# flanglet/kanzi

Hardware: AMD Instinct MI355X
Metric: encode+decode MB/s, 4 MiB-block synthetic stream, BWT+RANK+ZRLT & ANS0 (level-5 core chain), bit-exact .knz (higher is better)
Workload: dtype u8; 1 GPU; configs[2]: BWT+RANK+ZRLT & ANS0, 2048 x 4194304 B blocks per GPU per step (64 distinct synthetic blocks per GPU, SURVEY 8d generator standing in for silesia.tar, tiled), blocks round-robin over ranks; block_size=4194304, parallelism=blocks%1, round_trip_ok=True

## Files before the change

kanzi_amd/csrc/kz_ans.hip:

```cpp
#include "kz_device.h"
#include "kz_internal.h"
#include "kz_chunk.h"

typedef uint16_t u16;

#define ANS_TOP (1u << 15)
#define ANS_LR 12


struct BitW { u8* p; u32 pos; };
__device__ __forceinline__ void bw_put(BitW& w, u32 v, int count) {
  while (count > 0) {
    const int bitoff = w.pos & 7, room = 8 - bitoff;
    const int take = count < room ? count : room;
    const u32 bits = (v >> (count - take)) & ((1u << take) - 1u);
    w.p[w.pos >> 3] |= (u8)(bits << (room - take));
    w.pos += take; count -= take;
  }
}

typedef u16 __attribute__((aligned(1))) ans_u16_unaligned;
typedef u64 __attribute__((aligned(1))) ans_u64_unaligned;

__global__ __launch_bounds__(64) void k_ans_enc_chunk(const u8* __restrict__ src, int64_t stride,
                                                       const int32_t* __restrict__ d_len, AnsEnc E) {
  const int b = blockIdx.y, ck = blockIdx.x;
  const int count = d_len[b];
  const int lane = kz_lane();
  const int64_t ci = (int64_t)b * E.C + ck;
  const u8* blk = src + (int64_t)b * stride;
  u8* hdr = E.hdr + ci * ANS_HDR_BYTES;
  u8* scr = E.scr + ci * ANS_SCRATCH;
  if (count <= 32) {
    if (ck != 0) return;
    if (lane < count) scr[lane] = blk[lane];
    if (lane == 0) { E.hdrBits[ci] = 0; E.tailOff[ci] = 0; E.tailBits[ci] = 8u * (u32)count; }
    return;
  }
  const int start = ck * ANS_CHUNK;
  if (start >= count) return;
  const int end = min(count, start + ANS_CHUNK);
  const int len = end - start;

  __shared__ u32 hist[256];
  __shared__ u16 nfreq[256];
  __shared__ u8 alpha[256];
  __shared__ uint4 symTab[256];
  const u8* data = blk + start;
  __shared__ u32 hbuf[ANS_HDR_BYTES / 4];

  for (int i = lane; i < 256; i += 64) hist[i] = 0;
  for (int i = lane; i < ANS_HDR_BYTES / 4; i += 64) hbuf[i] = 0;
  __syncthreads();
  for (int i = lane * 4; i < len; i += 256) {
    u32 w = 0; int nb = min(4, len - i);
    if (nb == 4 && ((start + i) & 3) == 0) w = *(const u32*)(blk + start + i);
    else for (int k = 0; k < nb; k++) w |= (u32)blk[start + i + k] << (8 * k);
    for (int k = 0; k < 4; k++) {
      const bool valid = k < nb;
      const u32 c = (w >> (8 * k)) & 0xFF;
      const uint64_t peers = kz_match8(c, valid);
      if (valid && (peers & kz_lanemask_lt()) == 0) atomicAdd(&hist[c], (u32)__popcll(peers));
    }
  }
  __syncthreads();

  const u32 total = (u32)len, scale = 1u << ANS_LR;
  u32 f[4]; bool present[4];
  u32 alphabetSize = 0;
  u32 apos[4];
#pragma unroll
  for (int q = 0; q < 4; q++) {
    f[q] = hist[q * 64 + lane];
    present[q] = f[q] != 0;
    const uint64_t bal = kz_ballot(present[q]);
    apos[q] = alphabetSize + (u32)__popcll(bal & kz_lanemask_lt());
    alphabetSize += (u32)__popcll(bal);
    if (present[q]) alpha[apos[q]] = (u8)(q * 64 + lane);
  }
  if (total != scale) {
    u32 sumScaled = 0;
#pragma unroll
    for (int q = 0; q < 4; q++) {
      if (present[q]) {
        const u32 sf = f[q] * scale;
        f[q] = (sf <= total) ? 1u : (sf + (total >> 1)) / total;
      }
      sumScaled += kz_wave_sum(present[q] ? f[q] : 0);
    }
    if (alphabetSize == 1) {
#pragma unroll
      for (int q = 0; q < 4; q++) if (present[q]) f[q] = scale;
    } else if (sumScaled != scale) {
      u32 best = 0;
#pragma unroll
      for (int q = 0; q < 4; q++) { u32 v = present[q] ? f[q] : 0; best = max(best, v); }
#pragma unroll
      for (int d = 32; d > 0; d >>= 1) best = max(best, (u32)__shfl_xor(best, d, 64));
      int idxMax = 256;
#pragma unroll
      for (int q = 3; q >= 0; q--) {
        const uint64_t bal = kz_ballot(present[q] && f[q] == best);
        if (bal) idxMax = q * 64 + (int)__builtin_ctzll(bal);
      }
      int delta = (int)sumScaled - (int)scale;
      const int errThr = (int)(best >> 4);
      const int mq = idxMax >> 6, ml = idxMax & 63;
      int adjMax = 0;
      const int ad = delta < 0 ? -delta : delta;
      if (ad <= errThr) {
        adjMax = -delta;
      } else {
        if (delta < 0) { delta += errThr; adjMax = errThr; } else { delta -= errThr; adjMax = -errThr; }
#pragma unroll
        for (int q = 0; q < 4; q++) if (q == mq && lane == ml) f[q] = (u32)((int)f[q] + adjMax);
        adjMax = 0;
        const int inc = (delta > 0) ? -1 : 1;
        delta = delta < 0 ? -delta : delta;
        int round = 0;
        while ((++round < 6) && (delta > 0)) {
          int adjustments = 0;
#pragma unroll
          for (int q = 0; q < 4; q++) {
            const bool elig = present[q] && f[q] > 2;
            const uint64_t bal = kz_ballot(elig);
            const int pre = (int)__popcll(bal & kz_lanemask_lt());
            const int tot = (int)__popcll(bal);
            if (elig && pre < delta) f[q] = (u32)((int)f[q] + inc);
            const int used = tot < delta ? tot : delta;
            adjustments += used; delta -= used;
          }
          if (adjustments == 0) break;
        }
#pragma unroll
        for (int q = 0; q < 4; q++) if (q == mq && lane == ml) { int v = (int)f[q] - delta; f[q] = (u32)(v > 1 ? v : 1); }
      }
      if (adjMax != 0) {
#pragma unroll
        for (int q = 0; q < 4; q++) if (q == mq && lane == ml) f[q] = (u32)((int)f[q] + adjMax);
      }
    }
  }
  u32 cum = 0;
#pragma unroll
  for (int q = 0; q < 4; q++) {
    const u32 fv = present[q] ? f[q] : 0;
    const u32 inc = kz_wave_incl_sum(fv);
    const u32 cumFreq = cum + inc - fv;
    cum += __shfl(inc, 63, 64);
    const int s = q * 64 + lane;
    nfreq[s] = (u16)fv;
    if (present[q]) {
      u32 freq = fv;
      if (freq >= scale) freq = scale - 1;
      const u32 xmaxv = ((ANS_TOP >> ANS_LR) << 16) * freq;
      const u32 cmplv = scale - freq;
      if (freq < 2) symTab[s] = make_uint4(xmaxv, 0xFFFFFFFFu, cumFreq + scale - 1, cmplv | (32u << 16));
      else {
        int shift = 0;
        while (freq > (1u << shift)) shift++;
        symTab[s] = make_uint4(xmaxv, (u32)((((1ULL << (shift + 31)) + freq - 1) / freq) & 0xFFFFFFFFULL), cumFreq, cmplv | ((u32)(32 + shift - 1) << 16));
      }
    }
  }
  __syncthreads();
  u32 hb = 0;
  if (lane == 0) {
    BitW w{(u8*)hbuf, 0};
    bw_put(w, ANS_LR - 8, 3);
    if (alphabetSize == 256) { bw_put(w, 0, 1); bw_put(w, 0, 1); }
    else if (alphabetSize == 0) { bw_put(w, 0, 1); bw_put(w, 1, 1); }
    else {
      bw_put(w, 1, 1);
      const int lastMask = alpha[alphabetSize - 1] >> 3;
      bw_put(w, (u32)lastMask, 5);
      for (int i = 0; i <= lastMask; i++) {
        u32 m = 0;
        for (int j = 0; j < 8; j++) if (nfreq[i * 8 + j] != 0) m |= 1u << j;
        bw_put(w, m, 8);
      }
    }
    if (alphabetSize > 1) {
      const int chkSize = (alphabetSize >= 64) ? 8 : 6;
      int llr = 3;
      while ((1 << llr) <= ANS_LR) llr++;
      for (int i = 1; i < (int)alphabetSize; i += chkSize) {
        const int endj = (i + chkSize < (int)alphabetSize) ? i + chkSize : (int)alphabetSize;
        int mx = (int)nfreq[alpha[i]] - 1;
        for (int j = i + 1; j < endj; j++) { int v = (int)nfreq[alpha[j]] - 1; if (v > mx) mx = v; }
        int logMax = 0;
        while ((1 << logMax) <= mx) logMax++;
        bw_put(w, (u32)logMax, llr);
        if (logMax == 0) continue;
        for (int j = i; j < endj; j++) bw_put(w, (u32)nfreq[alpha[j]] - 1u, logMax);
      }
    }
    hb = w.pos;
    E.hdrBits[ci] = hb;
  }
  __syncthreads();
  for (int i = lane; i < ANS_HDR_BYTES / 4; i += 64) ((u32*)hdr)[i] = hbuf[i];
  if (alphabetSize <= 1) {
    if (lane == 0) { E.tailOff[ci] = 0; E.tailBits[ci] = 0; }
    return;
  }
  const int bufLen = ANS_SCRATCH;
  const int end4 = len & -4;
  int n = bufLen - 1;
  if (lane == 0) for (int i = len - 1; i >= end4; i--) scr[n - (len - 1 - i)] = data[i];
  n -= (len - end4);
  u32 st = ANS_TOP;
  int idx = n;
  if (lane < 4) {
#define ANS_ENC_STEP(WD)                                                                                      \
    { const u32 c = ((WD) >> (8 * (3 - lane))) & 0xFFu;                                                       \
      const uint4 sy = symTab[c];                                                                             \
      const bool x = st >= sy.x;                                               \
      const uint64_t bal = kz_ballot(x) & 0xFULL;                                                             \
      const int pre = (int)__popcll(bal & kz_lanemask_lt());                                                  \
      if (x) {                                                       \
        const int e = idx - 2 * pre;                                                                          \
        *(ans_u16_unaligned*)(scr + e - 1) = (u16)(((st & 0xFFu) << 8) | ((st >> 8) & 0xFFu));                \
        st >>= 16;                                                                                            \
      }                                                                                                       \
      idx -= 2 * (int)__popcll(bal);                                                                          \
      const u32 q = (u32)(((u64)st * (u64)sy.y) >> (sy.w >> 16));                                             \
      st = st + sy.z + q * (sy.w & 0xFFFFu); }
    const int T = end4 >> 2;
    const uint4* d16 = (const uint4*)data;
    int g = (T - 1) >> 2;
    uint4 cur = (T > 0) ? d16[g] : make_uint4(0, 0, 0, 0);
    for (; g >= 0; g--) {
      const uint4 nxt = (g > 0) ? d16[g - 1] : make_uint4(0, 0, 0, 0);
      const int top = min(3, T - 1 - 4 * g);
      if (top >= 3) ANS_ENC_STEP(cur.w)
      if (top >= 2) ANS_ENC_STEP(cur.z)
      if (top >= 1) ANS_ENC_STEP(cur.y)
      ANS_ENC_STEP(cur.x)
      cur = nxt;
    }
#undef ANS_ENC_STEP
  }
  idx = __shfl(idx, 0, 64);
  n = idx + 1;
  const u32 payload = (u32)(bufLen - n);
  u32 vlen = 1; { u32 v = payload; while (v >= 128) { v >>= 7; vlen++; } }
  const int tail = n - 16 - (int)vlen;
  if (lane == 0) {
    u32 v = payload; int p = tail;
    while (v >= 128) { scr[p++] = (u8)(0x80 | (v & 0x7F)); v >>= 7; }
    scr[p++] = (u8)v;
    E.tailOff[ci] = (u32)tail; E.tailBits[ci] = 8u * (payload + 16 + vlen);
  }
  if (lane < 4) {
    u8* p = scr + tail + vlen + 4 * lane;
    p[0] = (u8)(st >> 24); p[1] = (u8)(st >> 16); p[2] = (u8)(st >> 8); p[3] = (u8)st;
  }
}

__global__ __launch_bounds__(64) void k_ans_enc_scan(const int32_t* __restrict__ d_len, AnsEnc E, int64_t* __restrict__ d_bits, int rawLimit) {
  const int b = blockIdx.x;
  const int count = d_len[b];
  const int chunks = (count <= rawLimit) ? (count > 0 ? 1 : 0) : (count + E.chunk - 1) / E.chunk;
  const int lane = kz_lane();
  u64 carry = 0;
  for (int base = 0; base < chunks; base += 64) {
    const int c = base + lane;
    const int64_t ci = (int64_t)b * E.C + c;
    const u32 v = (c < chunks) ? E.hdrBits[ci] + E.tailBits[ci] : 0;
    const u32 inc = kz_wave_incl_sum(v);
    if (c < chunks) E.bitOff[ci] = carry + inc - v;
    carry += __shfl(inc, 63, 64);
  }
  if (lane == 0) d_bits[b] = (int64_t)carry;
}

__device__ __forceinline__ u32 kz_fetch32(const u8* __restrict__ p, int64_t nbits, int64_t r) {
  if (r >= nbits || r + 32 <= 0) return 0;
  u64 acc = 0;
  const int64_t byte0 = (r >= 0) ? (r >> 3) : -((-r + 7) >> 3);
  const int64_t nbytes = (nbits + 7) >> 3;
#pragma unroll
  for (int k = 0; k < 5; k++) {
    const int64_t bi = byte0 + k;
    const u64 v = (bi >= 0 && bi < nbytes) ? p[bi] : 0;
    acc = (acc << 8) | v;
  }
  const int sh = (int)(r - byte0 * 8);
  u32 w = (u32)((acc << sh) >> 8);
  const int64_t over = r + 32 - nbits;
  if (over > 0) w &= (over >= 32) ? 0u : (0xFFFFFFFFu << over);
  if (r < 0) { const int64_t under = -r; w &= (under >= 32) ? 0u : (0xFFFFFFFFu >> under); }
  return w;
}

__global__ __launch_bounds__(KZ_WG) void k_ans_enc_concat(const int32_t* __restrict__ d_len, AnsEnc E, u8* __restrict__ out,
                                                           int64_t outStride, const int32_t* __restrict__ d_hdrBytes, int rawLimit) {
  const int b = blockIdx.y, ck = blockIdx.x;
  const int count = d_len[b];
  const int chunks = (count <= rawLimit) ? (count > 0 ? 1 : 0) : (count + E.chunk - 1) / E.chunk;
  if (ck >= chunks) return;
  const int64_t ci = (int64_t)b * E.C + ck;
  const u8* hdr = E.hdr + ci * E.hdrStride;
  const int64_t hb = E.hdrBits[ci];
  const int64_t tb = (int64_t)E.tailBits[ci];
  const u8* tail = E.scr + ci * E.scrStride + E.tailOff[ci];
  const int64_t len = hb + tb;
  if (len == 0) return;
  const int64_t base = 8LL * d_hdrBytes[b] + (int64_t)E.bitOff[ci];
  u32* o = (u32*)(out + (int64_t)b * outStride);
  const int64_t wEnd = (base + len - 1) >> 5, wCap = (E.outCap >> 2) - 1;
  const int64_t w0 = base >> 5, w1 = wEnd < wCap ? wEnd : wCap;
  for (int64_t w = w0 + threadIdx.x; w <= w1; w += KZ_WG) {
    const int64_t r = w * 32 - base;
    u32 v = kz_fetch32(hdr, hb, r) | kz_fetch32(tail, tb, r - hb);
    v = __builtin_bswap32(v);
    if (r >= 0 && r + 32 <= len) o[w] = v; else atomicOr(&o[w], v);
  }
}

size_t kz_ans_scratch(int B, int maxN) {
  const int C = (maxN + 64) / ANS_CHUNK + 2;
  return (size_t)B * C * (ANS_HDR_BYTES + ANS_SCRATCH + 32) + (size_t)B * 64 + 8192;
}

int kz_chunk_enc_alloc(kz_ctx* ctx, kz_batch& bt, AnsEnc& E, int* chunksOut) {
  const int B = bt.B;
  int maxN = 0;
  for (int b = 0; b < B; b++) if (bt.h_len[b] > maxN) maxN = bt.h_len[b];
  E.C = (maxN + ANS_CHUNK - 1) / ANS_CHUNK + 1;
  E.hdr = (u8*)kz_arena_alloc(ctx, (size_t)B * E.C * ANS_HDR_BYTES);
  E.scr = (u8*)kz_arena_alloc(ctx, (size_t)B * E.C * ANS_SCRATCH);
  E.hdrBits = (u32*)kz_arena_alloc(ctx, (size_t)B * E.C * 4);
  E.tailOff = (u32*)kz_arena_alloc(ctx, (size_t)B * E.C * 4);
  E.tailBits = (u32*)kz_arena_alloc(ctx, (size_t)B * E.C * 4);
  E.bitOff = (u64*)kz_arena_alloc(ctx, (size_t)B * E.C * 8);
  if (!E.bitOff || !E.scr) { snprintf(ctx->err, sizeof(ctx->err), "entropy encode: arena overflow"); return -KZ_ERR_DEVICE; }
  KZ_HIP(hipMemsetAsync(E.hdrBits, 0, (size_t)B * E.C * 4, ctx->stream));
  KZ_HIP(hipMemsetAsync(E.tailBits, 0, (size_t)B * E.C * 4, ctx->stream));
  *chunksOut = (maxN + ANS_CHUNK - 1) / ANS_CHUNK;
  return 0;
}
int kz_chunk_enc_finish(kz_ctx* ctx, kz_batch& bt, AnsEnc& E, int chunks, uint8_t* out, int64_t outStride,
                        const int32_t* d_hdrBytes, int64_t* d_bits, int rawLimit) {
  const int B = bt.B;
  KZ_LAUNCH(ctx, KID_ANS_ENC_SCAN, k_ans_enc_scan, dim3(B), dim3(64), bt.d_len, E, d_bits, rawLimit);
  if (chunks > 0) KZ_LAUNCH(ctx, KID_ANS_ENC_CONCAT, k_ans_enc_concat, dim3(chunks, B), dim3(KZ_WG), bt.d_len, E, out, outStride, d_hdrBytes, rawLimit);
  KZ_HIP(hipGetLastError());
  return 0;
}

int kz_stage_ans0_encode(kz_ctx* ctx, kz_batch& bt, uint8_t* out, int64_t outStride, const int32_t* d_hdrBytes, int64_t* d_bits) {
  AnsEnc E; int chunks = 0;
  int rc = kz_chunk_enc_alloc(ctx, bt, E, &chunks);
  if (rc) return rc;
  if (chunks > 0) KZ_LAUNCH(ctx, KID_ANS_ENC_CHUNK, k_ans_enc_chunk, dim3(chunks, bt.B), dim3(64), bt.buf[bt.cur], bt.stride, bt.d_len, E);
  return kz_chunk_enc_finish(ctx, bt, E, chunks, out, outStride, d_hdrBytes, d_bits, 32);
}

#define ANS_EV_NONE 0x7FFFFFFF
#define ANS_EV_FAIL 0
#define ANS_EV_SKIP 1
#define ANS_EV_STOP 2
#define ANS_MAX_CHUNK_SIZE (1u << 27)
struct AnsDec {
  u64* chunkBit;
  int32_t* event;
  int32_t* nIdx;
  int32_t* hdrOnly;
  int C;
};

__device__ __forceinline__ u32 kz_peek(const u8* __restrict__ p, u64 pos, int count) {
  const u64 by = pos >> 3;
  u32 acc = ((u32)p[by] << 24) | ((u32)p[by + 1] << 16) | ((u32)p[by + 2] << 8) | (u32)p[by + 3];
  acc <<= (pos & 7);
  return count ? (acc >> (32 - count)) : 0;
}

__global__ void k_ans_dec_index(const u8* __restrict__ in, int64_t inStride, const int64_t* __restrict__ d_bitOff,
                                const int64_t* __restrict__ d_bitEnd, const int32_t* __restrict__ d_len, AnsDec D, int B, long long* __restrict__ endOut) {
  const int b = blockIdx.x * blockDim.x + threadIdx.x;
  if (b >= B) return;
  const int count = d_len[b];
  const u8* p = in + (int64_t)b * inStride;
  u64 pos = (u64)d_bitOff[b];
  const u64 endBits = (u64)d_bitEnd[b];
  int event = ANS_EV_NONE, nIdx = 0, bufLen = 0, hdrOnly = -1;
  if (count > 32) {
    const int chunks = (count + ANS_CHUNK - 1) / ANS_CHUNK;
    for (int c = 0; c < chunks; c++) {
      D.chunkBit[(int64_t)b * D.C + c] = pos;
      if (pos + 5 > endBits) { event = c * 4 + ANS_EV_FAIL; break; }
      const int lr = 8 + (int)kz_peek(p, pos, 3); pos += 3;
      int asz;
      if (kz_peek(p, pos, 1) == 0) { asz = (kz_peek(p, pos + 1, 1) == 1) ? 0 : 256; pos += 2; }
      else {
        const int lastMask = (int)kz_peek(p, pos + 1, 5); pos += 6;
        asz = 0;
        if (pos + 8ULL * (u64)(lastMask + 1) > endBits) { event = c * 4 + ANS_EV_FAIL; break; }
        for (int i = 0; i <= lastMask; i++) { asz += __popc(kz_peek(p, pos, 8)); pos += 8; }
      }
      if (asz == 0) { event = c * 4 + ANS_EV_FAIL; break; }
      {
        const int chkSize = (asz >= 64) ? 8 : 6;
        int llr = 3;
        while ((1 << llr) <= lr) llr++;
        for (int i = 1; i < asz && pos <= endBits; i += chkSize) {
          const int logMax = (int)kz_peek(p, pos, llr); pos += llr;
          const int endj = (i + chkSize < asz) ? i + chkSize : asz;
          pos += (u64)logMax * (u64)(endj - i);
        }
      }
      if (pos > endBits) { event = c * 4 + ANS_EV_FAIL; break; }
      nIdx = c + 1;
      if (asz == 1) continue;
      u32 v = kz_peek(p, pos, 8); pos += 8;
      u32 sz = v & 0x7F; int shift = 7;
      while (v >= 128) { v = kz_peek(p, pos, 8); pos += 8; sz |= (v & 0x7F) << shift; if (shift == 28) break; shift += 7; }
      if (sz >= ANS_MAX_CHUNK_SIZE) { hdrOnly = c; event = c * 4 + ANS_EV_SKIP; break; }
      const int clen = min(count - c * ANS_CHUNK, ANS_CHUNK);
      bufLen = max(bufLen, max(2 * clen, 256));
      if (sz > (u32)bufLen) { nIdx = c; event = c * 4 + ANS_EV_FAIL; break; }
      pos += 128 + 8ULL * sz;
      if (pos > endBits) { nIdx = c; event = c * 4 + ANS_EV_FAIL; break; }
    }
    if (event == ANS_EV_NONE) D.chunkBit[(int64_t)b * D.C + chunks] = pos;
  } else {
    pos += 8ULL * (u64)(count > 0 ? count : 0);
    if (pos > endBits) event = ANS_EV_FAIL;
  }
  if (endOut) endOut[b] = (long long)pos;
  D.event[b] = event;
  D.nIdx[b] = nIdx;
  D.hdrOnly[b] = hdrOnly;
}

__device__ __forceinline__ void ans_fill_f2s(const u16* __restrict__ cumf, u8* __restrict__ f2s, int scale, int lane) {
  const int x0 = lane * 64;
// ... 197 lines not shown
```

kanzi_amd/csrc/kz_api.hip:

```cpp
#include <dirent.h>
#include "kz_device.h"
#include "kz_internal.h"
#include <stdlib.h>
#include <algorithm>
#include <atomic>
#include <memory>
#include <thread>
#include <chrono>
#include <sched.h>

typedef uint32_t u32;
typedef uint8_t u8;
typedef unsigned long long u64;

extern "C" int32_t kz_abi_version(void) { return KZ_ABI_VERSION; }

extern "C" kz_ctx* kz_ctx_create(int32_t deviceId) {
  int ndev = 0;
  if (hipGetDeviceCount(&ndev) != hipSuccess || ndev <= 0) return nullptr;
  if (deviceId < 0 || deviceId >= ndev) return nullptr;
  if (hipSetDevice(deviceId) != hipSuccess) return nullptr;
  kz_ctx* ctx = new kz_ctx();
  ctx->device = deviceId;
  { int cus = 0; if (hipDeviceGetAttribute(&cus, hipDeviceAttributeMultiprocessorCount, deviceId) == hipSuccess && cus > 0) ctx->numCUs = cus; }
  if (hipStreamCreateWithFlags(&ctx->stream, hipStreamNonBlocking) != hipSuccess) { delete ctx; return nullptr; }
  if (hipHostMalloc((void**)&ctx->hpin, 1 << 20, hipHostMallocDefault) != hipSuccess) { hipStreamDestroy(ctx->stream); delete ctx; return nullptr; }
  ctx->hpinInts = (1 << 20) / 4;
  kz_switches_read(ctx->sw);
  {
    const int hw = (int)std::thread::hardware_concurrency();
    ctx->blockingWaits = ctx->sw.blockingWaits >= 0 ? ctx->sw.blockingWaits : ((hw > 0 && kz_usable_cpus() < hw) ? 1 : 0);
  }
  return ctx;
}
void kz_switches_read(kz_switches& s) {
  s = kz_switches();
  auto num = [](const char* name, int unset) { const char* e = getenv(name); return e ? atoi(e) : unset; };
  auto flag = [](const char* name) { return getenv(name) != nullptr ? 1 : 0; };
  auto digit = [](const char* name, int lo, int hi, int unset) { const char* e = getenv(name); return (e && e[0] >= '0' + lo && e[0] <= '0' + hi) ? e[0] - '0' : unset; };
  { const char* e = getenv("KZ_BLOCKING_WAITS"); s.blockingWaits = e ? (atoi(e) ? 1 : 0) : -1; }
  s.textGpu = digit("KZ_TEXT_GPU", 0, 3, -1);
  s.textGpuMin = num("KZ_TEXT_GPU_MIN", 512);
  s.textFwdGpu = digit("KZ_TEXT_FWD_GPU", 0, 1, -1);
  s.textFwdGpuMin = num("KZ_TEXT_FWD_GPU_MIN", 256);
  s.utfGpu = digit("KZ_UTF_GPU", 0, 0, 1);
  s.utfFwdGpu = digit("KZ_UTF_FWD_GPU", 0, 1, -1);
  s.textGpuTrace = flag("KZ_TEXT_GPU_TRACE");
  s.fuseMinBlocks = num("KZ_FUSE_MIN_BLOCKS", 32);
  s.overlapClasses = num("KZ_OVERLAP_CLASSES", 3);
  { const char* e = getenv("KZ_WIDE_QUEUES"); s.wideQueues = e ? (atoi(e) ? 1 : 0) : -1; }
  s.noSFirst = flag("KZ_NO_SFIRST");
  s.traceSched = flag("KZ_TRACE_SCHED");
  s.tracePipe = flag("KZ_TRACE_PIPE");
  s.hostChunk = num("KZ_HOST_CHUNK", 0);
  { const int v = num("KZ_HOST_CHUNK_DEC", 512); s.hostChunkDec = v < 8 ? 8 : v; }
  { const char* e = getenv("KZ_HOST_INV_STAGED"); s.hostInvStaged = e ? atoi(e) : -1; }
  s.streamChunk = num("KZ_STREAM_CHUNK", 0);
  s.streamSerial = flag("KZ_STREAM_SERIAL");
  s.bwtTrie = num("KZ_BWT_TRIE", -1); s.bwtTrieWin = num("KZ_BWT_TRIEWIN", -1); s.bwtBuckets = num("KZ_BWT_BUCKETS", -1);
  s.bwtDmax = num("KZ_BWT_DMAX", -1); s.bwtRetire = num("KZ_BWT_RETIRE", -1); s.bwtLazyRank = num("KZ_BWT_LAZYRANK", -1);
  s.bwtTrace = flag("KZ_BWT_TRACE");
  s.bwtTestTrieOverflow = digit("KZ_BWT_TEST_TRIE_OVERFLOW", 0, 9, -1);
  { const char* f = getenv("KZ_FPAQ_FORCE"); s.fpaqForce = f ? ((f[0] == 'w' || f[0] == 'W' || f[0] == '1') ? 1 : ((f[0] == 'l' || f[0] == 'L' || f[0] == '2') ? 2 : 0)) : 0; }
  s.sbrtForm = num("KZ_SBRT_FORM", -1);
}
extern "C" void kz_ctx_reload_switches(kz_ctx* ctx) {
  if (!ctx) return;
  kz_switches_read(ctx->sw);
  if (ctx->sw.blockingWaits >= 0) ctx->blockingWaits = ctx->sw.blockingWaits;
}
extern "C" void kz_ctx_destroy(kz_ctx* ctx) {
  if (!ctx) return;
  if (ctx->worker.joinable()) {
    { std::lock_guard<std::mutex> g(ctx->qmu); ctx->stopWorker = true; }
    ctx->qcv.notify_all();
    ctx->worker.join();
  }
  hipSetDevice(ctx->device);
  if (ctx->arena) hipFree(ctx->arena);
  for (int i = 0; i < 5; i++) { if (ctx->side[i]) hipStreamDestroy(ctx->side[i]); if (ctx->evJoin[i]) hipEventDestroy(ctx->evJoin[i]); }
  if (ctx->hpin) hipHostFree(ctx->hpin);
  for (int i = 0; i < 2; i++) {
    if (ctx->pinIn[i].p) hipHostFree(ctx->pinIn[i].p);
    if (ctx->pinOut[i].p) hipHostFree(ctx->pinOut[i].p);
    if (ctx->hsIn[i].p) hipHostFree(ctx->hsIn[i].p);
    if (ctx->hsOut[i].p) hipHostFree(ctx->hsOut[i].p);
    if (ctx->tfOut[i].p) hipHostFree(ctx->tfOut[i].p);
    if (ctx->hiAux[i].p) hipFree(ctx->hiAux[i].p);
    if (ctx->hiStream[i]) hipStreamDestroy(ctx->hiStream[i]);
    if (ctx->devIn[i].p) hipFree(ctx->devIn[i].p);
    if (ctx->devOut[i].p) hipFree(ctx->devOut[i].p);
  }
  if (ctx->tfIn.p) hipHostFree(ctx->tfIn.p);
  if (ctx->tfCopy) hipStreamDestroy(ctx->tfCopy);
  if (ctx->evBlock) hipEventDestroy(ctx->evBlock);
  if (ctx->copyUp) hipStreamDestroy(ctx->copyUp);
  if (ctx->copyDown) hipStreamDestroy(ctx->copyDown);
  if (ctx->stream) hipStreamDestroy(ctx->stream);
  delete ctx;
}
extern "C" int32_t kz_ctx_set_checksum(kz_ctx* ctx, int32_t bits) {
  if (!ctx || (bits != 0 && bits != 32 && bits != 64)) return -KZ_ERR_INVALID_PARAM;
  ctx->checksum = bits == 32 ? 1 : (bits == 64 ? 2 : 0);
  return 0;
}
extern "C" int32_t kz_ctx_set_skip_blocks(kz_ctx* ctx, int32_t on) {
  if (!ctx) return -KZ_ERR_INVALID_PARAM;
  ctx->skipBlocks = on ? 1 : 0;
  return 0;
}
extern "C" int32_t kz_ctx_set_data_type(kz_ctx* ctx, int32_t dataType) {
  if (!ctx || dataType < KZ_DT_UNDEFINED || dataType > KZ_DT_UTF8) return -KZ_ERR_INVALID_PARAM;
  ctx->dataType = dataType;
  return 0;
}
extern "C" int32_t kz_ctx_set_block_size(kz_ctx* ctx, int32_t blockSize) {
  if (!ctx || blockSize < 1024 || blockSize > (1 << 30) || (blockSize & 15)) return -KZ_ERR_BLOCK_SIZE;
  ctx->blockSize = blockSize;
  ctx->blockSizeSet = true;
  return 0;
}
extern "C" int32_t kz_ctx_set_entropy(kz_ctx* ctx, uint32_t entropyType) {
  if (!ctx || entropyType >= 9 || entropyType == 3) return -KZ_ERR_INVALID_CODEC;
  ctx->entropy = (int)entropyType;
  return 0;
}
extern "C" int32_t kz_ctx_reset(kz_ctx* ctx) {
  if (!ctx) return -KZ_ERR_INVALID_PARAM;
  ctx->checksum = 0; ctx->skipBlocks = 0; ctx->dataType = KZ_DT_UNDEFINED;
  ctx->blockSize = 4 * 1024 * 1024; ctx->blockSizeSet = false; ctx->entropy = KZ_E_NONE;
  return 0;
}
extern "C" int32_t kz_ctx_get_data_type(kz_ctx* ctx) { return ctx ? ctx->dataType : -KZ_ERR_INVALID_PARAM; }
extern "C" int32_t kz_pin_to_device_numa(int32_t deviceId) {
  char bdf[64] = {0};
  if (hipDeviceGetPCIBusId(bdf, (int)sizeof(bdf), deviceId) != hipSuccess) return -KZ_ERR_DEVICE;
  for (char* p = bdf; *p; p++) if (*p >= 'A' && *p <= 'F') *p = (char)(*p - 'A' + 'a');
  char path[160];
  snprintf(path, sizeof(path), "/sys/bus/pci/devices/%s/local_cpulist", bdf);
  FILE* f = fopen(path, "r");
  if (!f) return 0;
  char line[4096] = {0};
  const bool got = fgets(line, sizeof(line), f) != nullptr;
  fclose(f);
  if (!got) return 0;
  cpu_set_t set;
  CPU_ZERO(&set);
// ... 1899 lines not shown
```

kanzi_amd/csrc/kz_internal.h:

```cpp
#pragma once
#include <hip/hip_runtime.h>
#include <stdint.h>
#include <stdio.h>
#include <string.h>
#include <vector>
#include <condition_variable>
#include <deque>
#include <functional>
#include <map>
#include <set>
#include <mutex>
#include <thread>
#include "../../include/kanzi_hip.h"

enum KzKernelId { KID_ANS_ENC_CHUNK, KID_ANS_ENC_SCAN, KID_ANS_ENC_CONCAT, KID_ANS_DEC_INDEX, KID_ANS_DEC_CHUNK, KID_ANS_DEC_FIN, KID_MASK_LEN, KID_PASSTHROUGH, KID_FRAME_PREPARE, KID_COPY_BYTES, KID_FRAME_DECIDE, KID_FRAME_HEADER, KID_FRAME_PARSE, KID_COPY_PAYLOAD, KID_BWT_INIT, KID_RADIX_HIST, KID_RADIX_SCAN, KID_RADIX_SCATTER, KID_SEG_REDUCE, KID_SEG_SCAN, KID_SEG_APPLY, KID_LIVE_EMIT, KID_BWT_EMIT, KID_BWTI_PARSE, KID_BWTI_HIST, KID_BWTI_SCAN, KID_BWTI_SCATTER, KID_BWTI_WALK1, KID_BWTI_RESOLVE, KID_BWTI_COPY, KID_BWTI_LITERAL, KID_BWTI_FIN, KID_SBRT_LAST2, KID_SBRT_SCAN, KID_SBRT_REPLAY, KID_COPY_LEN, KID_SBRT_INVERSE, KID_ZRLT_F1, KID_ZRLT_F2, KID_ZRLT_F3, KID_ZRLT_FFIN, KID_ZRLT_I1, KID_ZRLT_I2, KID_ZRLT_I3, KID_ZRLT_IFIN, KID_RLT_F0, KID_RLT_FSCAN, KID_RLT_F1, KID_RLT_FSUM, KID_RLT_F3, KID_RLT_FTAIL, KID_RLT_I1, KID_RLT_ISCAN, KID_RLT_I2, KID_RLT_ISUM, KID_RLT_I3, KID_RLT_IFIN, KID_HUF_ENC_CHUNK, KID_HUF_DEC_INDEX, KID_HUF_DEC_CHUNK, KID_HUF_DEC_FIN, KID_FPAQ_ENC, KID_FPAQ_PACK, KID_FPAQ_DEC, KID_SRT_HIST, KID_SRT_PREP, KID_SRT_SCATTER, KID_SRT_INV, KID_LZ_FWD, KID_LZ_INV, KID_XXHASH, KID_BLOCK_MAGIC, KID_MM_ANALYZE, KID_MM_EMIT, KID_MM_CHECK, KID_MM_INV, KID_ALIAS_ANALYZE, KID_ALIAS_HIST1, KID_ALIAS_SELECT, KID_ALIAS_EMIT, KID_ALIAS_INV, KID_SKIP_DECIDE, KID_MSD_HIST, KID_MSD_SCAN, KID_MSD_SCATTER, KID_BUCKET_SORT, KID_BUCKET_COUNT, KID_BUCKET_COUNT_S, KID_TR_HIST16, KID_TR_ASSIGN, KID_TR_COUNT, KID_TR_SCATTER, KID_TR_SORT, KID_TEXT_INV, KID_UTF_INV, KID_TEXT_FWD, KID_TEXT_WALK, KID_UTF_FWD, KID_ANS1_HIST, KID_ANS1_NORM, KID_ANS1_HDR, KID_ANS1_ENC, KID_ANS1_DEC_INDEX, KID_ANS1_DEC_TABLE, KID_ANS1_DEC_CHUNK, KID_ANS1_DEC_FIN, KID_RANGE_ENC_CHUNK, KID_RANGE_ENC_FIN, KID_RANGE_DEC, KID_LZP_FWD, KID_LZP_INV, KID_EXE_SETUP, KID_EXE_MAP, KID_EXE_SCAN, KID_EXE_HIST, KID_EXE_DECIDE, KID_EXE_SIZE, KID_EXE_VERDICT, KID_EXE_EMIT, KID_COUNT };
#define KZ_KERNEL_NAMES { "k_ans_enc_chunk", "k_ans_enc_scan", "k_ans_enc_concat", "k_ans_dec_index", "k_ans_dec_chunk", "k_ans_dec_fin", "k_mask_len", "k_passthrough", "k_frame_prepare", "k_copy_bytes", "k_frame_decide", "k_frame_header", "k_frame_parse", "k_copy_payload", "k_bwt_init", "k_radix_hist", "k_radix_scan", "k_radix_scatter", "k_seg_reduce", "k_seg_scan", "k_seg_apply", "k_live_emit", "k_bwt_emit", "k_bwti_parse", "k_bwti_hist", "k_bwti_scan", "k_bwti_scatter", "k_bwti_walk1", "k_bwti_resolve", "k_bwti_copy", "k_bwti_literal", "k_bwti_fin", "k_sbrt_last2", "k_sbrt_scan", "k_sbrt_replay", "k_copy_len", "k_sbrt_inverse", "k_zrlt_f1", "k_zrlt_f2", "k_zrlt_f3", "k_zrlt_ffin", "k_zrlt_i1", "k_zrlt_i2", "k_zrlt_i3", "k_zrlt_ifin", "k_rlt_f0", "k_rlt_fscan", "k_rlt_f1", "k_rlt_fsum", "k_rlt_f3", "k_rlt_ftail", "k_rlt_i1", "k_rlt_iscan", "k_rlt_i2", "k_rlt_isum", "k_rlt_i3", "k_rlt_ifin", "k_huf_enc_chunk", "k_huf_dec_index", "k_huf_dec_chunk", "k_huf_dec_fin", "k_fpaq_enc", "k_fpaq_pack", "k_fpaq_dec", "k_srt_hist", "k_srt_prep", "k_srt_scatter", "k_srt_inv", "k_lz_fwd", "k_lz_inv", "k_xxhash", "k_block_magic", "k_mm_analyze", "k_mm_emit", "k_mm_check", "k_mm_inv", "k_alias_analyze", "k_alias_hist1", "k_alias_select", "k_alias_emit", "k_alias_inv", "k_skip_decide", "k_msd_hist", "k_msd_scan", "k_msd_scatter", "k_bucket_sort", "k_bucket_count", "k_bucket_count_s", "k_tr_hist16", "k_tr_assign", "k_tr_count", "k_tr_scatter", "k_tr_sort", "k_text_inv", "k_utf_inv", "k_text_fwd", "k_text_walk", "k_utf_fwd", "k_ans1_hist", "k_ans1_norm", "k_ans1_hdr", "k_ans1_enc", "k_ans1_dec_index", "k_ans1_dec_table", "k_ans1_dec_chunk", "k_ans1_dec_fin", "k_range_enc_chunk", "k_range_enc_fin", "k_range_dec", "k_lzp_fwd", "k_lzp_inv", "k_exe_setup", "k_exe_map", "k_exe_scan", "k_exe_hist", "k_exe_decide", "k_exe_size", "k_exe_verdict", "k_exe_emit" }
struct kz_switches {
  int blockingWaits = -1;
  int textGpu = -1;
  int textGpuMin = 512;
  int textFwdGpu = -1;
  int textFwdGpuMin = 256;
  int utfGpu = 1;
  int utfFwdGpu = -1;
  int textGpuTrace = 0;
  int fuseMinBlocks = 32;
  int overlapClasses = 3;
  int wideQueues = -1;
  int noSFirst = 0;
  int traceSched = 0;
  int tracePipe = 0;
  int hostChunk = 0;
  int hostChunkDec = 512;
  int hostInvStaged = -1;
  int streamChunk = 0;
  int streamSerial = 0;
  int bwtTrie = -1, bwtTrieWin = -1, bwtBuckets = -1, bwtDmax = -1, bwtRetire = -1;
  int bwtLazyRank = -1;
  int bwtTrace = 0;
  int bwtTestTrieOverflow = -1;
  int fpaqForce = 0;
  int sbrtForm = -1;
};
void kz_switches_read(kz_switches& s);

struct KzPending { hipEvent_t e0, e1; int id; };
struct kz_ctx {
  int device = 0;
  kz_switches sw;
  hipStream_t stream = nullptr;
  hipStream_t side[5] = {nullptr, nullptr, nullptr, nullptr, nullptr};
  hipEvent_t evJoin[5] = {nullptr, nullptr, nullptr, nullptr, nullptr};
  int wideQueues = -1;
  int wideNow = 0;
  uint8_t* arena = nullptr;
  size_t arenaCap = 0, arenaTop = 0;
  int32_t* hpin = nullptr;
  size_t hpinInts = 0;
  char err[512] = {0};
  float stageMs[KZ_MAX_STAGES] = {0};
  int64_t stageAlgBytes[KZ_MAX_STAGES] = {0};
  int nStages = 0;
  int checksum = 0;
  int skipBlocks = 0;
  int dataType = 0;
  int blockSize = 4 * 1024 * 1024;
  bool blockSizeSet = false;
  int entropy = KZ_E_NONE;
  int rltBlockSize = 0;
  int numCUs = 256;
  long long* d_endBits = nullptr;
  bool timing = false;
  bool ktiming = false;
  std::vector<KzPending> pending;
  std::vector<hipEvent_t> evPool;
  double kMs[KID_COUNT] = {0};
  double kMaxMs[KID_COUNT] = {0};
  long long kLaunches[KID_COUNT] = {0};
  std::thread worker;
  std::mutex qmu;
  std::condition_variable qcv;
  std::deque<std::pair<int64_t, std::function<int32_t()>>> queue;
  std::map<int64_t, int32_t> finished;
  std::set<int64_t> collected;
  int64_t collectedBelow = 1;
  int64_t nextJob = 1;
  bool stopWorker = false;
  struct Stage { uint8_t* p = nullptr; size_t cap = 0; };
  Stage pinIn[2], pinOut[2];
  Stage devIn[2], devOut[2];
  Stage hsIn[2], hsOut[2];
  Stage tfIn, tfOut[2];
  hipStream_t tfCopy = nullptr;
  hipStream_t copyUp = nullptr, copyDown = nullptr;
  Stage hiAux[2];
  hipStream_t hiStream[2] = {nullptr, nullptr};
  int blockingWaits = 0;
  hipEvent_t evBlock = nullptr;
};

struct kz_arena_guard { kz_ctx* c; size_t mark; ~kz_arena_guard() { c->arenaTop = mark; } };

#define KZ_HIP(x) do { hipError_t e_ = (x); if (e_ != hipSuccess) { \
  snprintf(ctx->err, sizeof(ctx->err), "%s:%d %s -> %s", __FILE__, __LINE__, #x, hipGetErrorString(e_)); \
  return -KZ_ERR_DEVICE; } } while (0)

static inline hipError_t kz_stream_sync(kz_ctx* ctx, hipStream_t st) {
  if (!ctx->blockingWaits) return hipStreamSynchronize(st);
  if (!ctx->evBlock) { hipError_t e = hipEventCreateWithFlags(&ctx->evBlock, hipEventBlockingSync | hipEventDisableTiming); if (e != hipSuccess) return e; }
  hipError_t e = hipEventRecord(ctx->evBlock, st);
  if (e != hipSuccess) return e;
  return hipEventSynchronize(ctx->evBlock);
}

#define KZ_MAX_PACKED_BLOCK ((1 << 24) - 257)
#define KZ_MAX_BLOCK ((1 << 30) + 1057)
#define KZ_MAX_BATCH 65535
int kz_hpin_reserve(kz_ctx* ctx, size_t ints);
static inline size_t kz_align(size_t v, size_t a) { return (v + a - 1) / a * a; }

int kz_arena_reserve(kz_ctx* ctx, size_t total);
void* kz_arena_alloc(kz_ctx* ctx, size_t bytes);

struct kz_batch {
  int B = 0;
// ... 111 lines not shown
```

Before: 4805 MB/s.

## Pack multiple ANS0 encode chunks per wavefront with 4-way interleaved lane groups

Adds k_ans_enc_pack, which handles K chunks per 64-lane workgroup. Each chunk is histogrammed, normalized and given a compact 8-byte symbol table in shared memory, and each header is written by a single lane through a 32-bit word accumulator. Encoding then runs 16 groups of 4 lanes, each group on its own chunk, with double-buffered 16-byte loads. The default (ansPack=-1) selects K=8, replacing the one-chunk-per-wave kernel. The aim is to cut launch count and idle lanes, at the cost of serial per-lane header emission and more shared memory.

```diff
diff --git a/kanzi_amd/csrc/kz_ans.hip b/kanzi_amd/csrc/kz_ans.hip
--- a/kanzi_amd/csrc/kz_ans.hip
+++ b/kanzi_amd/csrc/kz_ans.hip
@@ -21,6 +21,73 @@
 
 typedef u16 __attribute__((aligned(1))) ans_u16_unaligned;
 typedef u64 __attribute__((aligned(1))) ans_u64_unaligned;
+
+__device__ __forceinline__ void ans_normalize(u32 (&f)[4], const bool (&present)[4], const u32 alphabetSize, const u32 total, const int lane) {
+  const u32 scale = 1u << ANS_LR;
+  if (total != scale) {
+    u32 sumScaled = 0;
+#pragma unroll
+    for (int q = 0; q < 4; q++) {
+      if (present[q]) {
+        const u32 sf = f[q] * scale;
+        f[q] = (sf <= total) ? 1u : (sf + (total >> 1)) / total;
+      }
+      sumScaled += kz_wave_sum(present[q] ? f[q] : 0);
+    }
+    if (alphabetSize == 1) {
+#pragma unroll
+      for (int q = 0; q < 4; q++) if (present[q]) f[q] = scale;
+    } else if (sumScaled != scale) {
+      u32 best = 0;
+#pragma unroll
+      for (int q = 0; q < 4; q++) { u32 v = present[q] ? f[q] : 0; best = max(best, v); }
+#pragma unroll
+      for (int d = 32; d > 0; d >>= 1) best = max(best, (u32)__shfl_xor(best, d, 64));
+      int idxMax = 256;
+#pragma unroll
+      for (int q = 3; q >= 0; q--) {
+        const uint64_t bal = kz_ballot(present[q] && f[q] == best);
+        if (bal) idxMax = q * 64 + (int)__builtin_ctzll(bal);
+      }
+      int delta = (int)sumScaled - (int)scale;
+      const int errThr = (int)(best >> 4);
+      const int mq = idxMax >> 6, ml = idxMax & 63;
+      int adjMax = 0;
+      const int ad = delta < 0 ? -delta : delta;
+      if (ad <= errThr) {
+        adjMax = -delta;
+      } else {
+        if (delta < 0) { delta += errThr; adjMax = errThr; } else { delta -= errThr; adjMax = -errThr; }
+#pragma unroll
+        for (int q = 0; q < 4; q++) if (q == mq && lane == ml) f[q] = (u32)((int)f[q] + adjMax);
+        adjMax = 0;
+        const int inc = (delta > 0) ? -1 : 1;
+        delta = delta < 0 ? -delta : delta;
+        int round = 0;
+        while ((++round < 6) && (delta > 0)) {
+          int adjustments = 0;
+#pragma unroll
+          for (int q = 0; q < 4; q++) {
+            const bool elig = present[q] && f[q] > 2;
+            const uint64_t bal = kz_ballot(elig);
+            const int pre = (int)__popcll(bal & kz_lanemask_lt());
+            const int tot = (int)__popcll(bal);
+            if (elig && pre < delta) f[q] = (u32)((int)f[q] + inc);
+            const int used = tot < delta ? tot : delta;
+            adjustments += used; delta -= used;
+          }
+          if (adjustments == 0) break;
+        }
+#pragma unroll
+        for (int q = 0; q < 4; q++) if (q == mq && lane == ml) { int v = (int)f[q] - delta; f[q] = (u32)(v > 1 ? v : 1); }
+      }
+      if (adjMax != 0) {
+#pragma unroll
+        for (int q = 0; q < 4; q++) if (q == mq && lane == ml) f[q] = (u32)((int)f[q] + adjMax);
+      }
+    }
+  }
+}
 
 __global__ __launch_bounds__(64) void k_ans_enc_chunk(const u8* __restrict__ src, int64_t stride,
                                                        const int32_t* __restrict__ d_len, AnsEnc E) {
@@ -78,69 +145,7 @@
     alphabetSize += (u32)__popcll(bal);
     if (present[q]) alpha[apos[q]] = (u8)(q * 64 + lane);
   }
-  if (total != scale) {
-    u32 sumScaled = 0;
-#pragma unroll
-    for (int q = 0; q < 4; q++) {
-      if (present[q]) {
-        const u32 sf = f[q] * scale;
-        f[q] = (sf <= total) ? 1u : (sf + (total >> 1)) / total;
-      }
-      sumScaled += kz_wave_sum(present[q] ? f[q] : 0);
-    }
-    if (alphabetSize == 1) {
-#pragma unroll
-      for (int q = 0; q < 4; q++) if (present[q]) f[q] = scale;
-    } else if (sumScaled != scale) {
-      u32 best = 0;
-#pragma unroll
-      for (int q = 0; q < 4; q++) { u32 v = present[q] ? f[q] : 0; best = max(best, v); }
-#pragma unroll
-      for (int d = 32; d > 0; d >>= 1) best = max(best, (u32)__shfl_xor(best, d, 64));
-      int idxMax = 256;
-#pragma unroll
-      for (int q = 3; q >= 0; q--) {
-        const uint64_t bal = kz_ballot(present[q] && f[q] == best);
-        if (bal) idxMax = q * 64 + (int)__builtin_ctzll(bal);
-      }
-      int delta = (int)sumScaled - (int)scale;
-      const int errThr = (int)(best >> 4);
-      const int mq = idxMax >> 6, ml = idxMax & 63;
-      int adjMax = 0;
-      const int ad = delta < 0 ? -delta : delta;
-      if (ad <= errThr) {
-        adjMax = -delta;
-      } else {
-        if (delta < 0) { delta += errThr; adjMax = errThr; } else { delta -= errThr; adjMax = -errThr; }
-#pragma unroll
-        for (int q = 0; q < 4; q++) if (q == mq && lane == ml) f[q] = (u32)((int)f[q] + adjMax);
-        adjMax = 0;
-        const int inc = (delta > 0) ? -1 : 1;
-        delta = delta < 0 ? -delta : delta;
-        int round = 0;
-        while ((++round < 6) && (delta > 0)) {
-          int adjustments = 0;
-#pragma unroll
-          for (int q = 0; q < 4; q++) {
-            const bool elig = present[q] && f[q] > 2;
-            const uint64_t bal = kz_ballot(elig);
-            const int pre = (int)__popcll(bal & kz_lanemask_lt());
-            const int tot = (int)__popcll(bal);
-            if (elig && pre < delta) f[q] = (u32)((int)f[q] + inc);
-            const int used = tot < delta ? tot : delta;
-            adjustments += used; delta -= used;
-          }
-          if (adjustments == 0) break;
-        }
-#pragma unroll
-        for (int q = 0; q < 4; q++) if (q == mq && lane == ml) { int v = (int)f[q] - delta; f[q] = (u32)(v > 1 ? v : 1); }
-      }
-      if (adjMax != 0) {
-#pragma unroll
-        for (int q = 0; q < 4; q++) if (q == mq && lane == ml) f[q] = (u32)((int)f[q] + adjMax);
-      }
-    }
-  }
+  ans_normalize(f, present, alphabetSize, total, lane);
   u32 cum = 0;
 #pragma unroll
   for (int q = 0; q < 4; q++) {
@@ -258,6 +263,220 @@
   }
 }
 
+struct AnsHdrW { u32* p; u64 acc; int nb; u32 pos; };
+__device__ __forceinline__ void ans_hw_put(AnsHdrW& w, u32 v, int count) {
+  w.acc = (w.acc << count) | v; w.nb += count; w.pos += (u32)count;
+  if (w.nb >= 32) { w.nb -= 32; *w.p++ = __builtin_bswap32((u32)(w.acc >> w.nb)); }
+}
+
+template <int K>
+__global__ __launch_bounds__(64) void k_ans_enc_pack(const u8* __restrict__ src, int64_t stride,
+                                                      const int32_t* __restrict__ d_len, AnsEnc E) {
+  const int b = blockIdx.y, base = blockIdx.x * K;
+  const int count = d_len[b];
+  const int lane = kz_lane();
+  const u8* blk = src + (int64_t)b * stride;
+  if (count <= 32) {
+    if (base != 0) return;
+    const int64_t ci = (int64_t)b * E.C;
+    if (lane < count) E.scr[ci * ANS_SCRATCH + lane] = blk[lane];
+    if (lane == 0) { E.hdrBits[ci] = 0; E.tailOff[ci] = 0; E.tailBits[ci] = 8u * (u32)count; }
+    return;
+  }
+  const int nChunks = (count + ANS_CHUNK - 1) / ANS_CHUNK;
+  if (base >= nChunks) return;
+  const int ng = min(K, nChunks - base);
+
+  __shared__ uint2 symTab[K][256];
+  __shared__ u64 pres[K][4];
+
+  const u32 scale = 1u << ANS_LR;
+  const int grp = lane >> 2, l4 = lane & 3;
+  for (int g = 0; g < ng; g++) {
+    const int start = (base + g) * ANS_CHUNK;
+    const int len = min(count, start + ANS_CHUNK) - start;
+    const u8* data = blk + start;
+    u32* hist = (u32*)symTab[g];
+    for (int i = lane; i < 512; i += 64) hist[i] = 0;
+    __syncthreads();
+    u32* hl = hist + (lane & 1);
+    for (int i = lane * 16; i < len; i += 1024) {
+      if (i + 16 <= len) {
+        const uint4 v = *(const uint4*)(data + i);
+#pragma unroll
+        for (int k = 0; k < 4; k++) {
+          atomicAdd(hl + 2 * ((v.x >> (8 * k)) & 0xFFu), 1u); atomicAdd(hl + 2 * ((v.y >> (8 * k)) & 0xFFu), 1u);
+          atomicAdd(hl + 2 * ((v.z >> (8 * k)) & 0xFFu), 1u); atomicAdd(hl + 2 * ((v.w >> (8 * k)) & 0xFFu), 1u);
+        }
+      } else {
+        for (int k = i; k < len; k++) atomicAdd(hl + 2 * (u32)data[k], 1u);
+      }
+    }
+    __syncthreads();
+    u32 f[4]; bool present[4];
+    u32 alphabetSize = 0;
+#pragma unroll
+    for (int q = 0; q < 4; q++) {
+      const uint2 h = *(const uint2*)(hist + 2 * (q * 64 + lane));
+      f[q] = h.x + h.y;
+      present[q] = f[q] != 0;
+      const uint64_t bal = kz_ballot(present[q]);
+      alphabetSize += (u32)__popcll(bal);
+      if (lane == 0) pres[g][q] = bal;
+    }
+    __syncthreads();
+    ans_normalize(f, present, alphabetSize, (u32)len, lane);
+    u32 cum = 0;
+#pragma unroll
+    for (int q = 0; q < 4; q++) {
+      const u32 fv = present[q] ? f[q] : 0;
+      const u32 inc = kz_wave_incl_sum(fv);
+      const u32 cumFreq = cum + inc - fv;
+      cum += __shfl(inc, 63, 64);
+      if (present[q]) {
+        u32 freq = fv;
+        if (freq >= scale) freq = scale - 1;
+        if (freq < 2) symTab[g][q * 64 + lane] = make_uint2(0xFFFFFFFFu, freq | ((cumFreq + scale - 1) << 12));
+        else {
+          int shift = 0;
+          while (freq > (1u << shift)) shift++;
+          symTab[g][q * 64 + lane] = make_uint2((u32)((((1ULL << (shift + 31)) + freq - 1) / freq) & 0xFFFFFFFFULL), freq | (cumFreq << 12) | ((u32)(shift - 1) << 25));
+        }
+      }
+    }
+  }
+  __syncthreads();
+
+  if (lane < ng) {
+    const int64_t ci = (int64_t)b * E.C + base + lane;
+    const uint2* tab = symTab[lane];
+    const u64* pr = pres[lane];
+    const int asz = (int)(__popcll(pr[0]) + __popcll(pr[1]) + __popcll(pr[2]) + __popcll(pr[3]));
+    AnsHdrW w{(u32*)(E.hdr + ci * ANS_HDR_BYTES), 0, 0, 0};
+    ans_hw_put(w, ANS_LR - 8, 3);
+    if (asz == 256) { ans_hw_put(w, 0, 1); ans_hw_put(w, 0, 1); }
+    else if (asz == 0) { ans_hw_put(w, 0, 1); ans_hw_put(w, 1, 1); }
+    else {
+      ans_hw_put(w, 1, 1);
+      int top = 3;
+      while (pr[top] == 0) top--;
+      const int lastMask = (top * 64 + 63 - (int)__builtin_clzll(pr[top])) >> 3;
+      ans_hw_put(w, (u32)lastMask, 5);
+      for (int i = 0; i <= lastMask; i++) ans_hw_put(w, (u32)(pr[i >> 3] >> (8 * (i & 7))) & 0xFFu, 8);
+    }
+    if (asz > 1) {
+      const int chkSize = (asz >= 64) ? 8 : 6;
+      int llr = 3;
+      while ((1 << llr) <= ANS_LR) llr++;
+      int wd = 0;
+      u64 bits = pr[0];
+      while (bits == 0) bits = pr[++wd];
+      bits &= bits - 1;
+      auto next = [&](u64& bs, int& wi) -> u32 {
+        while (bs == 0) bs = pr[++wi];
+        const int s = wi * 64 + (int)__builtin_ctzll(bs);
+        bs &= bs - 1;
+        return (tab[s].y & 0xFFFu) - 1u;
+      };
+      for (int i = 1; i < asz; i += chkSize) {
+        const int cnt = min(chkSize, asz - i);
+        u64 bits2 = bits; int wd2 = wd;
+        u32 mx = 0;
+        for (int j = 0; j < cnt; j++) mx = max(mx, next(bits2, wd2));
+        const int logMax = 32 - __clz(mx);
+        ans_hw_put(w, (u32)logMax, llr);
+        if (logMax != 0) for (int j = 0; j < cnt; j++) ans_hw_put(w, next(bits, wd), logMax);
+        else { bits = bits2; wd = wd2; }
+      }
+    }
+    if (w.nb > 0) *w.p = __builtin_bswap32((u32)(w.acc << (32 - w.nb)));
+    E.hdrBits[ci] = w.pos;
+    if (asz <= 1) { E.tailOff[ci] = 0; E.tailBits[ci] = 0; }
+  }
+
+  bool act = grp < ng;
+  int len = 0;
+  if (act) {
+    const int start = (base + grp) * ANS_CHUNK;
+    len = min(count, start + ANS_CHUNK) - start;
+    const u64* pr = pres[grp];
+    act = (__popcll(pr[0]) + __popcll(pr[1]) + __popcll(pr[2]) + __popcll(pr[3])) > 1;
+  }
+  const int gq = act ? grp : 0;
+  const int64_t ci = (int64_t)b * E.C + base + gq;
+  const u8* data = blk + (int64_t)(base + gq) * ANS_CHUNK;
+  u8* scr = E.scr + ci * ANS_SCRATCH;
+  const uint2* tab = symTab[gq];
+  const int bufLen = ANS_SCRATCH;
+  const int end4 = len & -4;
+  int n = bufLen - 1;
+  if (act && l4 < len - end4) scr[n - l4] = data[len - 1 - l4];
+  n -= (len - end4);
+  u32 st = ANS_TOP;
+  int idx = n;
+  const int T = act ? (end4 >> 2) : 0;
+  int Tmax = T;
+#pragma unroll
+  for (int d = 32; d > 0; d >>= 1) Tmax = max(Tmax, __shfl_xor(Tmax, d, 64));
+  Tmax = __builtin_amdgcn_readfirstlane(Tmax);
+  if (Tmax > 0) {
+    const int sh8 = 8 * (3 - l4), gsh = lane & 60;
+    const u32 lt = (1u << l4) - 1u;
+#define ANS_PACK_STEP(WD)                                                                                     \
+    { const u32 c = ((WD) >> sh8) & 0xFFu;                                                                    \
+      const uint2 sy = tab[c];                                                                                \
+      const u32 fq = sy.y & 0xFFFu;                                                                           \
+      const bool x = st >= (fq << 19);                                  \
+      const u32 gb = (u32)(kz_ballot(x) >> gsh) & 0xFu;                                                       \
+      if (x) {                                                       \
+        const int e = idx - 2 * (int)__popc(gb & lt);                                                         \
+        *(ans_u16_unaligned*)(scr + e - 1) = (u16)(((st & 0xFFu) << 8) | ((st >> 8) & 0xFFu));                \
+        st >>= 16;                                                                                            \
+      }                                                                                                       \
+      idx -= 2 * (int)__popc(gb);                                                                             \
+      const u32 q = __umulhi(st, sy.x) >> (sy.y >> 25);                                                       \
+      st = st + ((sy.y >> 12) & 0x1FFFu) + q * (scale - fq); }
+#define ANS_PACK_LOAD(V, G)                                                                                   \
+    { _Pragma("unroll") for (int m = 0; m < 4; m++) { V[m] = make_uint4(0, 0, 0, 0); if (16 * (G) + 4 * m < T) V[m] = d16[4 * (G) + m]; } }
+#define ANS_PACK_STEP4(V, W0)                                                                                 \
+    { if ((W0) + 3 < T) ANS_PACK_STEP(V.w)                                                                    \
+      if ((W0) + 2 < T) ANS_PACK_STEP(V.z)                                                                    \
+      if ((W0) + 1 < T) ANS_PACK_STEP(V.y)                                                                    \
+      if ((W0) < T) ANS_PACK_STEP(V.x) }
+    const uint4* d16 = (const uint4*)data;
+    int g = (Tmax - 1) >> 4;
+    uint4 cur[4], nxt[4];
+    ANS_PACK_LOAD(cur, g)
+    __builtin_amdgcn_s_waitcnt(0x0F70);
+    for (; g >= 0; g--) {
+      if (g > 0) ANS_PACK_LOAD(nxt, g - 1)
+      const int w0 = 16 * g;
+      ANS_PACK_STEP4(cur[3], w0 + 12)
+      ANS_PACK_STEP4(cur[2], w0 + 8)
+      ANS_PACK_STEP4(cur[1], w0 + 4)
+      ANS_PACK_STEP4(cur[0], w0)
+#pragma unroll
+      for (int m = 0; m < 4; m++) cur[m] = nxt[m];
+    }
+#undef ANS_PACK_STEP4
+#undef ANS_PACK_LOAD
+#undef ANS_PACK_STEP
+  }
+  if (!act) return;
+  n = idx + 1;
+  const u32 payload = (u32)(bufLen - n);
+  u32 vlen = 1; { u32 v = payload; while (v >= 128) { v >>= 7; vlen++; } }
+  const int tail = n - 16 - (int)vlen;
+  if (l4 == 0) {
+    u32 v = payload; int p = tail;
+    while (v >= 128) { scr[p++] = (u8)(0x80 | (v & 0x7F)); v >>= 7; }
+    scr[p++] = (u8)v;
+    E.tailOff[ci] = (u32)tail; E.tailBits[ci] = 8u * (payload + 16 + vlen);
+  }
+  u8* p = scr + tail + vlen + 4 * l4;
+  p[0] = (u8)(st >> 24); p[1] = (u8)(st >> 16); p[2] = (u8)(st >> 8); p[3] = (u8)st;
+}
+
 __global__ __launch_bounds__(64) void k_ans_enc_scan(const int32_t* __restrict__ d_len, AnsEnc E, int64_t* __restrict__ d_bits, int rawLimit) {
   const int b = blockIdx.x;
   const int count = d_len[b];
@@ -354,7 +573,13 @@
   AnsEnc E; int chunks = 0;
   int rc = kz_chunk_enc_alloc(ctx, bt, E, &chunks);
   if (rc) return rc;
-  if (chunks > 0) KZ_LAUNCH(ctx, KID_ANS_ENC_CHUNK, k_ans_enc_chunk, dim3(chunks, bt.B), dim3(64), bt.buf[bt.cur], bt.stride, bt.d_len, E);
+  if (chunks > 0) {
+    const int k = ctx->sw.ansPack;
+    if (k == 0) KZ_LAUNCH(ctx, KID_ANS_ENC_CHUNK, k_ans_enc_chunk, dim3(chunks, bt.B), dim3(64), bt.buf[bt.cur], bt.stride, bt.d_len, E);
+    else if (k == 4) KZ_LAUNCH(ctx, KID_ANS_ENC_CHUNK, k_ans_enc_pack<4>, dim3((chunks + 3) / 4, bt.B), dim3(64), bt.buf[bt.cur], bt.stride, bt.d_len, E);
+    else if (k == 16) KZ_LAUNCH(ctx, KID_ANS_ENC_CHUNK, k_ans_enc_pack<16>, dim3((chunks + 15) / 16, bt.B), dim3(64), bt.buf[bt.cur], bt.stride, bt.d_len, E);
+    else KZ_LAUNCH(ctx, KID_ANS_ENC_CHUNK, k_ans_enc_pack<8>, dim3((chunks + 7) / 8, bt.B), dim3(64), bt.buf[bt.cur], bt.stride, bt.d_len, E);
+  }
   return kz_chunk_enc_finish(ctx, bt, E, chunks, out, outStride, d_hdrBytes, d_bits, 32);
 }
 
diff --git a/kanzi_amd/csrc/kz_api.hip b/kanzi_amd/csrc/kz_api.hip
--- a/kanzi_amd/csrc/kz_api.hip
+++ b/kanzi_amd/csrc/kz_api.hip
@@ -63,6 +63,7 @@
   s.bwtTestTrieOverflow = digit("KZ_BWT_TEST_TRIE_OVERFLOW", 0, 9, -1);
   { const char* f = getenv("KZ_FPAQ_FORCE"); s.fpaqForce = f ? ((f[0] == 'w' || f[0] == 'W' || f[0] == '1') ? 1 : ((f[0] == 'l' || f[0] == 'L' || f[0] == '2') ? 2 : 0)) : 0; }
   s.sbrtForm = num("KZ_SBRT_FORM", -1);
+  { const int v = num("KZ_ANS_PACK", -1); s.ansPack = (v == 0 || v == 4 || v == 8 || v == 16) ? v : -1; }
 }
 extern "C" void kz_ctx_reload_switches(kz_ctx* ctx) {
   if (!ctx) return;
diff --git a/kanzi_amd/csrc/kz_internal.h b/kanzi_amd/csrc/kz_internal.h
--- a/kanzi_amd/csrc/kz_internal.h
+++ b/kanzi_amd/csrc/kz_internal.h
@@ -41,6 +41,7 @@
   int bwtTestTrieOverflow = -1;
   int fpaqForce = 0;
   int sbrtForm = -1;
+  int ansPack = -1;
 };
 void kz_switches_read(kz_switches& s);
 
```

Result: no change. 4802 MB/s (-0.1%).
